# mindspore-lab/mindaudio

Measured on AMD Instinct MI355X. Metric: utterances/s (16 kHz×10 s) fbanks+Conformer fwd, 1/2/4/8 MI355X, higher is better.
Workload: dtype bf16; 1 GPU; features.fbank (n_fft=512 hop=160 n_mels=80, batch-global top_db) on 64 x (10 s @16 kHz) synthetic waves per GPU -> Conformer-small encoder forward (12 blocks, d=256, 4 heads, ff=2048, conv k=15, eval mode) on the (64, 1000, 80) features; random-init weights; global_batch=64, frames=1000

## Files before the change

mindaudio_amd/csrc/subsample_fused.hip:

```cpp
#include <hip/hip_runtime.h>
#include <stdint.h>
#include <stdlib.h>

#include <type_traits>
#include <utility>

#include "../../include/mindaudio_amd.h"

#include "launch.h"

namespace ma {

typedef __attribute__((ext_vector_type(8))) __bf16 sf_bf16x8;
typedef __attribute__((ext_vector_type(4))) float sf_f32x4;
typedef __attribute__((ext_vector_type(2))) __bf16 sf_bf16x2;
typedef __attribute__((ext_vector_type(2))) float sf_f32x2;
typedef __attribute__((address_space(3))) void sf_lds_void_t;

template <int... Is, class F>
__device__ __forceinline__ void sf_static_for_impl(std::integer_sequence<int, Is...>, F&& f) {
  (f(std::integral_constant<int, Is>{}), ...);
}
template <int N, class F>
__device__ __forceinline__ void sf_static_for(F&& f) {
  sf_static_for_impl(std::make_integer_sequence<int, N>{}, f);
}

constexpr int kSfRows = 128, kSfC = 256, kSfThreads = 512;
constexpr int kSfIdim = 80, kSfF1 = 39, kSfF2 = 19;
constexpr int kSfNhoMax = 8;
constexpr int kSfH1Max = 2 * kSfNhoMax + 1;
constexpr int kSfInMax = 2 * kSfH1Max + 1;
constexpr int kSfPosMax = 672;
constexpr int kSfPitch = 80;
constexpr int kSfChunks = 8, kSfTaps = 9;
constexpr int kSfW2Bytes = kSfC * 9 * kSfC * 2;
constexpr int kSfOffX = 11264;
constexpr int kSfOffPatch = kSfOffX + kSfPosMax * 64;
constexpr int kSfPatchBytes = kSfPosMax * kSfPitch;
constexpr int kSfLds = kSfOffPatch + 2 * kSfPatchBytes;
constexpr int kSfOutPitch = 144;
static_assert(kSfInMax * kSfIdim <= 6 * kSfThreads && kSfPosMax <= 2 * kSfThreads && kSfLds <= 163840, "tile geometry");
static_assert(4 * kSfRows * kSfOutPitch <= kSfOffPatch + kSfPatchBytes, "epilogue staging must not reach patch buffer 1");

struct SubsampleFusedParams {
  const float* x;
  int64_t sb, st, sf;
  const float *mean, *istd;
  const char* packed;
  const float* b1;
  const float* b2;
  uint16_t* out;
  int32_t Ho, tiles_per_utt;
};

__device__ __forceinline__ uint32_t sf_pack_bf16(float lo, float hi) {
  const sf_bf16x2 r = __builtin_convertvector((sf_f32x2){lo, hi}, sf_bf16x2);
  return *reinterpret_cast<const uint32_t*>(&r);
}
__device__ __forceinline__ float sf_head(float x) { return __uint_as_float(sf_pack_bf16(x, 0.0f) << 16); }

template <bool IS_W>
__device__ __forceinline__ void sf_split_row(const float (&v)[9], uint32_t (&d)[16]) {
  float h[9], l[9];
#pragma unroll
  for (int t = 0; t < 9; ++t) {
    h[t] = sf_head(v[t]);
    l[t] = v[t] - h[t];
  }
  float k[32];
#pragma unroll
  for (int t = 0; t < 9; ++t) {
    k[t] = h[t];
    k[9 + t] = IS_W ? l[t] : h[t];
    k[18 + t] = IS_W ? h[t] : l[t];
  }
#pragma unroll
  for (int t = 27; t < 32; ++t) k[t] = 0.0f;
#pragma unroll
  for (int j = 0; j < 16; ++j) d[j] = sf_pack_bf16(k[2 * j], k[2 * j + 1]);
}

__global__ void subsample_fused_pack_kernel(const uint16_t* __restrict__ w2, const float* __restrict__ w1, uint4* __restrict__ out) {
  const int idx = blockIdx.x * blockDim.x + threadIdx.x;
  constexpr int kN2 = 4 * kSfChunks * kSfTaps * 4 * 64;
  if (idx < kN2) {
    const int lane = idx & 63, jt = (idx >> 6) & 3, ft = (idx >> 8) % (kSfChunks * kSfTaps), wv = (idx >> 8) / (kSfChunks * kSfTaps);
    const int cc = ft / kSfTaps, tap = ft - cc * kSfTaps;
    const int n = 64 * wv + 16 * jt + (lane & 15);
    out[idx] = *reinterpret_cast<const uint4*>(w2 + (int64_t)n * (9 * kSfC) + tap * kSfC + 32 * cc + 8 * (lane >> 4));
  } else if (idx < kN2 + 16 * 64) {
    const int j = idx - kN2, lane = j & 63, item = j >> 6;
    const int ch = 16 * item + (lane & 15), g = lane >> 4;
    float v[9];
#pragma unroll
    for (int t = 0; t < 9; ++t) v[t] = w1[ch * 9 + t];
    uint32_t d[16];
    sf_split_row<true>(v, d);
    out[idx] = g == 0 ? make_uint4(d[0], d[1], d[2], d[3]) : g == 1 ? make_uint4(d[4], d[5], d[6], d[7])
             : g == 2 ? make_uint4(d[8], d[9], d[10], d[11]) : make_uint4(d[12], d[13], d[14], d[15]);
  }
}

#ifndef SF_PRIO_C
#define SF_PRIO_C 1
#endif
#ifndef SF_PRIO_P
#define SF_PRIO_P 0
#endif
#ifdef MA_SF_PROF
__device__ unsigned long long g_sf_prof[2 * 3 * 32];
#define SF_STAMP(k) do { asm volatile("s_waitcnt lgkmcnt(0)" ::: "memory"); sf_ts[(k)] = __builtin_amdgcn_s_memtime(); asm volatile("s_waitcnt lgkmcnt(0)" ::: "memory"); } while (0)
#define SF_FLUSH(role)                                                                                        \
  do {                                                                                                        \
    const int slot_ = blockIdx.x == 0 ? 0 : blockIdx.x == 1200 ? 1 : blockIdx.x == 2300 ? 2 : -1;             \
    if (slot_ >= 0 && lane == 0)                                                                              \
      for (int k_ = 0; k_ < 32; ++k_) g_sf_prof[((role) * 3 + slot_) * 32 + k_] = sf_ts[k_];                  \
  } while (0)
#else
#define SF_STAMP(k) do { } while (0)
#define SF_FLUSH(role) do { } while (0)
#endif

__global__ __launch_bounds__(kSfThreads, 2) void subsample_fused_kernel(const SubsampleFusedParams p) {
  extern __shared__ __attribute__((aligned(16))) char smem[];
#ifdef MA_SF_PROF
  unsigned long long sf_ts[32] = {};
#endif
  SF_STAMP(0);
  const int tid = threadIdx.x, lane = tid & 63;
  const int wave = __builtin_amdgcn_readfirstlane(tid >> 6);
  const int b = blockIdx.x / p.tiles_per_utt, ti = blockIdx.x - b * p.tiles_per_utt;
  const int npos = p.Ho * kSfF2;
  const int p0 = ti * kSfRows;
  const int np = min(kSfRows, npos - p0);
  const int ho0 = p0 / kSfF2;
  const int nho = (p0 + np - 1) / kSfF2 - ho0 + 1;
  const int nh1 = 2 * nho + 1, nin = 2 * nh1 + 1;
  const int npatch = nh1 * kSfF1;
  float* rows = reinterpret_cast<float*>(smem);
  char* xim = smem + kSfOffX;
  char* patch = smem + kSfOffPatch;

  {
    const float* xb = p.x + (int64_t)b * p.sb + (int64_t)(4 * ho0) * p.st;
    const bool tfast = p.st <= p.sf;
    const int n = nin * kSfIdim;
    float v[6], mu[6], is[6];
    int dst[6];
#pragma unroll
    for (int j = 0; j < 6; ++j) {
      const int i = min(tid + kSfThreads * j, n - 1);
      const int r = tfast ? i % nin : i / kSfIdim, f = tfast ? i / nin : i % kSfIdim;
      dst[j] = r * kSfIdim + f;
      v[j] = xb[r * p.st + f * p.sf];
      mu[j] = p.mean ? p.mean[f] : 0.0f;
      is[j] = p.mean ? p.istd[f] : 1.0f;
    }
#pragma unroll
    for (int j = 0; j < 6; ++j)
      if (tid + kSfThreads * j < n) rows[dst[j]] = p.mean ? (v[j] - mu[j]) * is[j] : v[j];
  }
  __syncthreads();
  SF_STAMP(1);
#pragma unroll
  for (int j = 0; j < 2; ++j) {
    const int pos = tid + kSfThreads * j;
    if (pos < kSfPosMax) {
      uint32_t d[16];
      if (pos < npatch) {
        const int h = pos / kSfF1, w = pos - h * kSfF1;
        const float* in = rows + (2 * h) * kSfIdim + 2 * w;
        float v[9];
#pragma unroll
        for (int kh = 0; kh < 3; ++kh)
#pragma unroll
          for (int kw = 0; kw < 3; ++kw) v[kh * 3 + kw] = in[kh * kSfIdim + kw];
        sf_split_row<false>(v, d);
      } else {
#pragma unroll
        for (int q = 0; q < 16; ++q) d[q] = 0u;
      }
      uint4* xo = reinterpret_cast<uint4*>(xim + pos * 64);
      xo[0] = make_uint4(d[0], d[1], d[2], d[3]);
      xo[1] = make_uint4(d[4], d[5], d[6], d[7]);
      xo[2] = make_uint4(d[8], d[9], d[10], d[11]);
      xo[3] = make_uint4(d[12], d[13], d[14], d[15]);
    }
  }
  __syncthreads();
  SF_STAMP(2);

  const int ci = lane & 15, gi = lane >> 4;
  auto build_patch = [&](int cc, int pw, int nprod) __attribute__((always_inline)) {
    const uint4* w1f = reinterpret_cast<const uint4*>(p.packed + kSfW2Bytes) + (2 * cc) * 64 + lane;
    const uint4 wa = w1f[0], wb = w1f[64];
    const sf_bf16x8 a0 = *reinterpret_cast<const sf_bf16x8*>(&wa), a1 = *reinterpret_cast<const sf_bf16x8*>(&wb);
    const float4 ba = *reinterpret_cast<const float4*>(p.b1 + 32 * cc + 4 * gi);
    const float4 bb = *reinterpret_cast<const float4*>(p.b1 + 32 * cc + 16 + 4 * gi);
    const sf_f32x4 c0 = {ba.x, ba.y, ba.z, ba.w}, c1 = {bb.x, bb.y, bb.z, bb.w};
    const char* xsrc = xim + ci * 64 + gi * 16;
    char* dst = patch + (cc & 1) * kSfPatchBytes + ci * kSfPitch + gi * 8;
    const int ntile = (npatch + 15) >> 4;
    for (int pt = pw; pt < ntile; pt += nprod) {
      const uint4 xr = *reinterpret_cast<const uint4*>(xsrc + pt * (16 * 64));
      const sf_bf16x8 xf = *reinterpret_cast<const sf_bf16x8*>(&xr);
      const sf_f32x4 d0 = __builtin_amdgcn_mfma_f32_16x16x32_bf16(a0, xf, c0, 0, 0, 0);
      const sf_f32x4 d1 = __builtin_amdgcn_mfma_f32_16x16x32_bf16(a1, xf, c1, 0, 0, 0);
      char* o = dst + pt * (16 * kSfPitch);
      *reinterpret_cast<uint2*>(o) = make_uint2(sf_pack_bf16(fmaxf(d0[0], 0.f), fmaxf(d0[1], 0.f)), sf_pack_bf16(fmaxf(d0[2], 0.f), fmaxf(d0[3], 0.f)));
      *reinterpret_cast<uint2*>(o + 32) = make_uint2(sf_pack_bf16(fmaxf(d1[0], 0.f), fmaxf(d1[1], 0.f)), sf_pack_bf16(fmaxf(d1[2], 0.f), fmaxf(d1[3], 0.f)));
    }
  };
  build_patch(0, wave, 8);
  SF_STAMP(3);

  if (wave >= 4) {
#if SF_PRIO_P
    __builtin_amdgcn_s_setprio(SF_PRIO_P);
#endif
#pragma unroll 1
    for (int k = 0; k + 1 < kSfChunks; ++k) {
      __syncthreads();
      SF_STAMP(4 + 2 * k);
      build_patch(k + 1, wave - 4, 4);
      SF_STAMP(5 + 2 * k);
    }
    __syncthreads();
    SF_STAMP(20);
    if (wave == 4) SF_FLUSH(1);
    return;
  }

#if SF_PRIO_C
  __builtin_amdgcn_s_setprio(SF_PRIO_C);
#endif
  const int c = lane & 15, g = lane >> 4;
  uint32_t a_addr[8];
#pragma unroll
  for (int s = 0; s < 8; ++s) {
    int m = 16 * s + c;
    if (m >= np) m = np - 1;
    const int pos = p0 + m, ho = pos / kSfF2, wo = pos - ho * kSfF2;
    a_addr[s] = (uint32_t)(uintptr_t)(sf_lds_void_t*)(patch + ((2 * (ho - ho0)) * kSfF1 + 2 * wo) * kSfPitch + g * 16);
  }
  const uint32_t voff = lane * 16 + 2048;
  const char* wbase = p.packed + (int64_t)wave * (kSfChunks * kSfTaps) * 4096;
#define SF_LOAD(dst, ft, jt)                                                                                          \
  do {                                                                                                                \
    const char* cb_ = wbase + (int64_t)((ft) < kSfChunks * kSfTaps ? (ft) : kSfChunks * kSfTaps - 1) * 4096;          \
    asm volatile("global_load_dwordx4 %0, %1, %2 offset:%3" : "=v"(dst) : "v"(voff), "s"(cb_), "n"(((jt) - 2) * 1024) \
                 : "memory");                                                                                         \
  } while (0)
  sf_bf16x8 ring[8];
  sf_f32x4 acc[4][8];
  sf_bf16x8 af[2][8];
#define SF_LDS(dst, s_, imm_) asm volatile("ds_read_b128 %0, %1 offset:%2" : "=v"(dst) : "v"(a_addr[s_]), "n"(imm_) : "memory")
#define SF_LDS8(buf_, imm_)                                                                                   \
  SF_LDS(af[buf_][0], 0, imm_); SF_LDS(af[buf_][1], 1, imm_); SF_LDS(af[buf_][2], 2, imm_); SF_LDS(af[buf_][3], 3, imm_); \
  SF_LDS(af[buf_][4], 4, imm_); SF_LDS(af[buf_][5], 5, imm_); SF_LDS(af[buf_][6], 6, imm_); SF_LDS(af[buf_][7], 7, imm_)
  auto tap_step = [&](auto tapc, auto parc, auto bufc, int ft) __attribute__((always_inline)) {
    constexpr int TAP = decltype(tapc)::value, PAR = decltype(parc)::value, BUF = decltype(bufc)::value;
    constexpr int IMM = BUF * kSfPatchBytes + ((TAP / 3) * kSfF1 + (TAP % 3)) * kSfPitch;
    constexpr int NTAP = TAP + 1;
    constexpr int IMM_N = BUF * kSfPatchBytes + ((NTAP / 3) * kSfF1 + (NTAP % 3)) * kSfPitch;
    if constexpr (TAP == 0) { SF_LDS8(PAR, IMM); }
    if constexpr (TAP < kSfTaps - 1) {
      SF_LDS8(PAR ^ 1, IMM_N);
      asm volatile("s_waitcnt lgkmcnt(8)"
                   : "+v"(af[PAR][0]), "+v"(af[PAR][1]), "+v"(af[PAR][2]), "+v"(af[PAR][3]), "+v"(af[PAR][4]), "+v"(af[PAR][5]),
                     "+v"(af[PAR][6]), "+v"(af[PAR][7])::"memory");
    } else {
      asm volatile("s_waitcnt lgkmcnt(0)"
                   : "+v"(af[PAR][0]), "+v"(af[PAR][1]), "+v"(af[PAR][2]), "+v"(af[PAR][3]), "+v"(af[PAR][4]), "+v"(af[PAR][5]),
                     "+v"(af[PAR][6]), "+v"(af[PAR][7])::"memory");
    }
    sf_static_for<4>([&](auto tc) __attribute__((always_inline)) {
      constexpr int jt = decltype(tc)::value;
      constexpr int q = PAR * 4 + jt;
      asm volatile("s_waitcnt vmcnt(7)" : "+v"(ring[q])::"memory");
      sf_static_for<8>([&](auto sc) __attribute__((always_inline)) {
        constexpr int s = decltype(sc)::value;
        acc[jt][s] = __builtin_amdgcn_mfma_f32_16x16x32_bf16(ring[q], af[PAR][s], acc[jt][s], 0, 0, 0);
      });
      __builtin_amdgcn_sched_barrier(0);
      SF_LOAD(ring[q], ft + 2, jt);
    });
  };
  auto chunk_mfma = [&](auto bufc, int cc) __attribute__((always_inline)) {
    constexpr int BUF = decltype(bufc)::value;
    sf_static_for<kSfTaps>([&](auto tapc) __attribute__((always_inline)) {
      constexpr int TAP = decltype(tapc)::value;
      tap_step(tapc, std::integral_constant<int, (BUF + TAP) & 1>{}, bufc, cc * kSfTaps + TAP);
    });
  };

#pragma unroll
  for (int jt = 0; jt < 4; ++jt)
#pragma unroll
    for (int s = 0; s < 8; ++s) acc[jt][s] = sf_f32x4{0.f, 0.f, 0.f, 0.f};
  SF_LOAD(ring[0], 0, 0); SF_LOAD(ring[1], 0, 1); SF_LOAD(ring[2], 0, 2); SF_LOAD(ring[3], 0, 3);
  SF_LOAD(ring[4], 1, 0); SF_LOAD(ring[5], 1, 1); SF_LOAD(ring[6], 1, 2); SF_LOAD(ring[7], 1, 3);
  asm volatile("s_waitcnt lgkmcnt(0)" ::: "memory");
  __builtin_amdgcn_s_barrier();
#ifdef MA_SF_PROF
#pragma unroll
#else
#pragma unroll 1
#endif
  for (int cc = 0; cc < kSfChunks; cc += 2) {
    SF_STAMP(4 + 2 * cc);
    chunk_mfma(std::integral_constant<int, 0>{}, cc);
    SF_STAMP(5 + 2 * cc);
    __builtin_amdgcn_s_barrier();
    SF_STAMP(6 + 2 * cc);
    chunk_mfma(std::integral_constant<int, 1>{}, cc + 1);
    SF_STAMP(7 + 2 * cc);
    if (cc + 2 < kSfChunks) __builtin_amdgcn_s_barrier();
  }
  asm volatile("s_waitcnt vmcnt(0)"
               : "+v"(ring[0]), "+v"(ring[1]), "+v"(ring[2]), "+v"(ring[3]), "+v"(ring[4]), "+v"(ring[5]), "+v"(ring[6]), "+v"(ring[7])
               :
               : "memory");
#undef SF_LOAD
#undef SF_LDS
#undef SF_LDS8
  SF_STAMP(20);

  char* strip = smem + wave * (kSfRows * kSfOutPitch);
  float4 bv[4];
#pragma unroll
  for (int jt = 0; jt < 4; ++jt) bv[jt] = *reinterpret_cast<const float4*>(p.b2 + 64 * wave + 16 * jt + 4 * g);
#pragma unroll
  for (int s = 0; s < 8; ++s) {
    char* srow = strip + (16 * s + c) * kSfOutPitch + 8 * g;
#pragma unroll
    for (int jt = 0; jt < 4; ++jt) {
      const float v0 = fmaxf(acc[jt][s][0] + bv[jt].x, 0.f), v1 = fmaxf(acc[jt][s][1] + bv[jt].y, 0.f);
      const float v2 = fmaxf(acc[jt][s][2] + bv[jt].z, 0.f), v3 = fmaxf(acc[jt][s][3] + bv[jt].w, 0.f);
      *reinterpret_cast<uint2*>(srow + 32 * jt) = make_uint2(sf_pack_bf16(v0, v1), sf_pack_bf16(v2, v3));
    }
  }
  uint16_t* obase = p.out + ((int64_t)b * npos + p0) * kSfC + 64 * wave + 8 * (lane & 7);
#pragma unroll
  for (int it = 0; it < 16; ++it) {
    const int m = 8 * it + (lane >> 3);
    const uint4 v = *reinterpret_cast<const uint4*>(strip + m * kSfOutPitch + 16 * (lane & 7));
    if (m < np) *reinterpret_cast<uint4*>(obase + (int64_t)m * kSfC) = v;
  }
  SF_STAMP(21);
  if (wave == 0) SF_FLUSH(0);
}

#ifdef MA_SF_PROF
extern "C" int ma_debug_sf_prof(unsigned long long* host192) {
  return hipMemcpyFromSymbol(host192, HIP_SYMBOL(g_sf_prof), sizeof(unsigned long long) * 192) == hipSuccess ? 0 : -1;
}
#endif

MA_LDS_ATTR(subsample_fused_kernel, kSfLds);

}

using namespace ma;

extern "C" int64_t ma_subsample_fused_packed_bytes(int64_t idim, int64_t C) {
  if (idim != kSfIdim || C != kSfC) return MA_ERR_UNSUPPORTED;
  return (int64_t)kSfW2Bytes + 16 * 1024;
}

extern "C" int ma_subsample_fused_pack_bf16(const float* W1, const void* W2, int64_t idim, int64_t C, void* packed, ma_stream_t stream) {
  if (!W1 || !W2 || !packed) return MA_ERR_INVALID_ARG;
  if (ma_subsample_fused_packed_bytes(idim, C) < 0) return MA_ERR_UNSUPPORTED;
  if ((reinterpret_cast<uintptr_t>(W2) | reinterpret_cast<uintptr_t>(packed)) & 15) return MA_ERR_INVALID_ARG;
  const int total = 4 * kSfChunks * kSfTaps * 4 * 64 + 16 * 64;
  MA_LAUNCH(subsample_fused_pack_kernel, dim3((total + 255) / 256), dim3(256), 0, (hipStream_t)stream,
            reinterpret_cast<const uint16_t*>(W2), W1, reinterpret_cast<uint4*>(packed));
  return MA_OK;
}

extern "C" int ma_subsample_fused_bf16(const float* x, int64_t stride_b, int64_t stride_t, int64_t stride_f, int64_t batch, int64_t T,
                                       int32_t idim, const float* cmvn_mean, const float* cmvn_istd, const void* packed, const float* b1,
                                       const float* b2, int64_t C, void* out, ma_stream_t stream) {
  if (!x || !packed || !b1 || !b2 || !out || batch < 1 || T < 7) return MA_ERR_INVALID_ARG;
  if ((cmvn_mean == nullptr) != (cmvn_istd == nullptr)) return MA_ERR_INVALID_ARG;
  if (ma_subsample_fused_packed_bytes(idim, C) < 0) return MA_ERR_UNSUPPORTED;
  if ((reinterpret_cast<uintptr_t>(packed) | reinterpret_cast<uintptr_t>(out) | reinterpret_cast<uintptr_t>(b2) |
       reinterpret_cast<uintptr_t>(b1)) & 15)
    return MA_ERR_INVALID_ARG;
  const int64_t T1 = (T - 3) / 2 + 1, Ho = (T1 - 3) / 2 + 1;
  const int64_t tiles = (Ho * kSfF2 + kSfRows - 1) / kSfRows;
  if (batch * tiles > 0x7fffffff || Ho > (1 << 24)) return MA_ERR_UNSUPPORTED;
  SubsampleFusedParams p;
  p.x = x;
  p.sb = stride_b;
  p.st = stride_t;
  p.sf = stride_f;
  p.mean = cmvn_mean;
  p.istd = cmvn_istd;
  p.packed = reinterpret_cast<const char*>(packed);
  p.b1 = b1;
  p.b2 = b2;
  p.out = reinterpret_cast<uint16_t*>(out);
  p.Ho = (int32_t)Ho;
  p.tiles_per_utt = (int32_t)tiles;
  MA_LAUNCH(subsample_fused_kernel, dim3((unsigned)(batch * tiles)), dim3(kSfThreads), kSfLds, (hipStream_t)stream, p);
  return MA_OK;
}
```

Measured before the change: 33050 utterances/s.

## Make fused subsample conv a persistent kernel overlapping next-tile load with MFMA

Replaces the one-block-per-tile subsample conv kernel with a persistent kernel launched at most once per CU. Each block walks a contiguous range of 16-row granules, so tile sizes are balanced across blocks. The producer waves load and normalise the next tile's input rows while still building patches for the current tile, and the consumer waves keep their weight ring loads flowing across tiles. The second conv's bias is staged in LDS and the epilogue is written in two halves. This aims to cut launch tail imbalance and the per-tile prologue stalls, at the cost of more register pressure and more complex synchronisation. The old tile kernel stays available behind an environment variable.

```diff
diff --git a/mindaudio_amd/csrc/subsample_fused.hip b/mindaudio_amd/csrc/subsample_fused.hip
--- a/mindaudio_amd/csrc/subsample_fused.hip
+++ b/mindaudio_amd/csrc/subsample_fused.hip
@@ -52,6 +52,8 @@
   const float* b2;
   uint16_t* out;
   int32_t Ho, tiles_per_utt;
+  int32_t gran_per_utt;
+  int64_t gran_total;
 };
 
 __device__ __forceinline__ uint32_t sf_pack_bf16(float lo, float hi) {
@@ -79,6 +81,99 @@
   for (int t = 27; t < 32; ++t) k[t] = 0.0f;
 #pragma unroll
   for (int j = 0; j < 16; ++j) d[j] = sf_pack_bf16(k[2 * j], k[2 * j + 1]);
+}
+
+struct SfGeom {
+  int ho0, nin, npatch;
+};
+__device__ __forceinline__ SfGeom sf_geom(int p0, int np) {
+  const int ho0 = p0 / kSfF2;
+  const int nho = (p0 + np - 1) / kSfF2 - ho0 + 1;
+  const int nh1 = 2 * nho + 1;
+  return {ho0, 2 * nh1 + 1, nh1 * kSfF1};
+}
+
+template <int J>
+struct SfRowsRegs {
+  float v[J], mu[J], is[J];
+  int dst[J];
+};
+template <int NT, int J>
+__device__ __forceinline__ void sf_rows_load(const SubsampleFusedParams& p, int b, const SfGeom& q, int t, SfRowsRegs<J>& r) {
+  static_assert(kSfInMax * kSfIdim <= NT * J, "rows staging");
+  const float* xb = p.x + (int64_t)b * p.sb + (int64_t)(4 * q.ho0) * p.st;
+  const bool tfast = p.st <= p.sf;
+  const int n = q.nin * kSfIdim;
+#pragma unroll
+  for (int j = 0; j < J; ++j) {
+    const int i = min(t + NT * j, n - 1);
+    const int rr = tfast ? i % q.nin : i / kSfIdim, f = tfast ? i / q.nin : i % kSfIdim;
+    r.dst[j] = rr * kSfIdim + f;
+    r.v[j] = xb[rr * p.st + f * p.sf];
+    r.mu[j] = p.mean ? p.mean[f] : 0.0f;
+    r.is[j] = p.mean ? p.istd[f] : 1.0f;
+  }
+}
+template <int NT, int J>
+__device__ __forceinline__ void sf_rows_store(const SubsampleFusedParams& p, const SfGeom& q, int t, const SfRowsRegs<J>& r, float* rows) {
+  const int n = q.nin * kSfIdim;
+#pragma unroll
+  for (int j = 0; j < J; ++j)
+    if (t + NT * j < n) rows[r.dst[j]] = p.mean ? (r.v[j] - r.mu[j]) * r.is[j] : r.v[j];
+}
+
+__device__ __forceinline__ void sf_build_x(const float* rows, char* xim, int pos, int npatch) {
+  uint32_t d[16];
+  if (pos < npatch) {
+    const int h = pos / kSfF1, w = pos - h * kSfF1;
+    const float* in = rows + (2 * h) * kSfIdim + 2 * w;
+    float v[9];
+#pragma unroll
+    for (int kh = 0; kh < 3; ++kh)
+#pragma unroll
+      for (int kw = 0; kw < 3; ++kw) v[kh * 3 + kw] = in[kh * kSfIdim + kw];
+    sf_split_row<false>(v, d);
+  } else {
+#pragma unroll
+    for (int q = 0; q < 16; ++q) d[q] = 0u;
+  }
+  uint4* xo = reinterpret_cast<uint4*>(xim + pos * 64);
+  xo[0] = make_uint4(d[0], d[1], d[2], d[3]);
+  xo[1] = make_uint4(d[4], d[5], d[6], d[7]);
+  xo[2] = make_uint4(d[8], d[9], d[10], d[11]);
+  xo[3] = make_uint4(d[12], d[13], d[14], d[15]);
+}
+
+struct SfW1 {
+  sf_bf16x8 a0, a1;
+  sf_f32x4 c0, c1;
+};
+__device__ __forceinline__ SfW1 sf_patch_w1(const SubsampleFusedParams& p, int cc, int lane) {
+  const int gi = lane >> 4;
+  const uint4* w1f = reinterpret_cast<const uint4*>(p.packed + kSfW2Bytes) + (2 * cc) * 64 + lane;
+  const uint4 wa = w1f[0], wb = w1f[64];
+  const float4 ba = *reinterpret_cast<const float4*>(p.b1 + 32 * cc + 4 * gi);
+  const float4 bb = *reinterpret_cast<const float4*>(p.b1 + 32 * cc + 16 + 4 * gi);
+  return {*reinterpret_cast<const sf_bf16x8*>(&wa), *reinterpret_cast<const sf_bf16x8*>(&wb), sf_f32x4{ba.x, ba.y, ba.z, ba.w},
+          sf_f32x4{bb.x, bb.y, bb.z, bb.w}};
+}
+__device__ __forceinline__ void sf_build_patch(const SfW1& w, const char* xim, char* patch, int npatch, int cc, int pw, int nprod,
+                                               int lane) {
+  const int ci = lane & 15, gi = lane >> 4;
+  const sf_bf16x8 a0 = w.a0, a1 = w.a1;
+  const sf_f32x4 c0 = w.c0, c1 = w.c1;
+  const char* xsrc = xim + ci * 64 + gi * 16;
+  char* dst = patch + (cc & 1) * kSfPatchBytes + ci * kSfPitch + gi * 8;
+  const int ntile = (npatch + 15) >> 4;
+  for (int pt = pw; pt < ntile; pt += nprod) {
+    const uint4 xr = *reinterpret_cast<const uint4*>(xsrc + pt * (16 * 64));
+    const sf_bf16x8 xf = *reinterpret_cast<const sf_bf16x8*>(&xr);
+    const sf_f32x4 d0 = __builtin_amdgcn_mfma_f32_16x16x32_bf16(a0, xf, c0, 0, 0, 0);
+    const sf_f32x4 d1 = __builtin_amdgcn_mfma_f32_16x16x32_bf16(a1, xf, c1, 0, 0, 0);
+    char* o = dst + pt * (16 * kSfPitch);
+    *reinterpret_cast<uint2*>(o) = make_uint2(sf_pack_bf16(fmaxf(d0[0], 0.f), fmaxf(d0[1], 0.f)), sf_pack_bf16(fmaxf(d0[2], 0.f), fmaxf(d0[3], 0.f)));
+    *reinterpret_cast<uint2*>(o + 32) = make_uint2(sf_pack_bf16(fmaxf(d1[0], 0.f), fmaxf(d1[1], 0.f)), sf_pack_bf16(fmaxf(d1[2], 0.f), fmaxf(d1[3], 0.f)));
+  }
 }
 
 __global__ void subsample_fused_pack_kernel(const uint16_t* __restrict__ w2, const float* __restrict__ w1, uint4* __restrict__ out) {
@@ -122,7 +217,7 @@
 #define SF_FLUSH(role) do { } while (0)
 #endif
 
-__global__ __launch_bounds__(kSfThreads, 2) void subsample_fused_kernel(const SubsampleFusedParams p) {
+__global__ __launch_bounds__(kSfThreads, 2) void subsample_fused_tile_kernel(const SubsampleFusedParams p) {
   extern __shared__ __attribute__((aligned(16))) char smem[];
 #ifdef MA_SF_PROF
   unsigned long long sf_ts[32] = {};
@@ -134,85 +229,26 @@
   const int npos = p.Ho * kSfF2;
   const int p0 = ti * kSfRows;
   const int np = min(kSfRows, npos - p0);
-  const int ho0 = p0 / kSfF2;
-  const int nho = (p0 + np - 1) / kSfF2 - ho0 + 1;
-  const int nh1 = 2 * nho + 1, nin = 2 * nh1 + 1;
-  const int npatch = nh1 * kSfF1;
+  const SfGeom q = sf_geom(p0, np);
+  const int npatch = q.npatch;
   float* rows = reinterpret_cast<float*>(smem);
   char* xim = smem + kSfOffX;
   char* patch = smem + kSfOffPatch;
 
   {
-    const float* xb = p.x + (int64_t)b * p.sb + (int64_t)(4 * ho0) * p.st;
-    const bool tfast = p.st <= p.sf;
-    const int n = nin * kSfIdim;
-    float v[6], mu[6], is[6];
-    int dst[6];
-#pragma unroll
-    for (int j = 0; j < 6; ++j) {
-      const int i = min(tid + kSfThreads * j, n - 1);
-      const int r = tfast ? i % nin : i / kSfIdim, f = tfast ? i / nin : i % kSfIdim;
-      dst[j] = r * kSfIdim + f;
-      v[j] = xb[r * p.st + f * p.sf];
-      mu[j] = p.mean ? p.mean[f] : 0.0f;
-      is[j] = p.mean ? p.istd[f] : 1.0f;
-    }
-#pragma unroll
-    for (int j = 0; j < 6; ++j)
-      if (tid + kSfThreads * j < n) rows[dst[j]] = p.mean ? (v[j] - mu[j]) * is[j] : v[j];
+    SfRowsRegs<6> r;
+    sf_rows_load<kSfThreads, 6>(p, b, q, tid, r);
+    sf_rows_store<kSfThreads, 6>(p, q, tid, r, rows);
   }
   __syncthreads();
   SF_STAMP(1);
 #pragma unroll
-  for (int j = 0; j < 2; ++j) {
-    const int pos = tid + kSfThreads * j;
-    if (pos < kSfPosMax) {
-      uint32_t d[16];
-      if (pos < npatch) {
-        const int h = pos / kSfF1, w = pos - h * kSfF1;
-        const float* in = rows + (2 * h) * kSfIdim + 2 * w;
-        float v[9];
-#pragma unroll
-        for (int kh = 0; kh < 3; ++kh)
-#pragma unroll
-          for (int kw = 0; kw < 3; ++kw) v[kh * 3 + kw] = in[kh * kSfIdim + kw];
-        sf_split_row<false>(v, d);
-      } else {
-#pragma unroll
-        for (int q = 0; q < 16; ++q) d[q] = 0u;
-      }
-      uint4* xo = reinterpret_cast<uint4*>(xim + pos * 64);
-      xo[0] = make_uint4(d[0], d[1], d[2], d[3]);
-      xo[1] = make_uint4(d[4], d[5], d[6], d[7]);
-      xo[2] = make_uint4(d[8], d[9], d[10], d[11]);
-      xo[3] = make_uint4(d[12], d[13], d[14], d[15]);
-    }
-  }
+  for (int j = 0; j < 2; ++j)
+    if (tid + kSfThreads * j < kSfPosMax) sf_build_x(rows, xim, tid + kSfThreads * j, npatch);
   __syncthreads();
   SF_STAMP(2);
 
-  const int ci = lane & 15, gi = lane >> 4;
-  auto build_patch = [&](int cc, int pw, int nprod) __attribute__((always_inline)) {
-    const uint4* w1f = reinterpret_cast<const uint4*>(p.packed + kSfW2Bytes) + (2 * cc) * 64 + lane;
-    const uint4 wa = w1f[0], wb = w1f[64];
-    const sf_bf16x8 a0 = *reinterpret_cast<const sf_bf16x8*>(&wa), a1 = *reinterpret_cast<const sf_bf16x8*>(&wb);
-    const float4 ba = *reinterpret_cast<const float4*>(p.b1 + 32 * cc + 4 * gi);
-    const float4 bb = *reinterpret_cast<const float4*>(p.b1 + 32 * cc + 16 + 4 * gi);
-    const sf_f32x4 c0 = {ba.x, ba.y, ba.z, ba.w}, c1 = {bb.x, bb.y, bb.z, bb.w};
-    const char* xsrc = xim + ci * 64 + gi * 16;
-    char* dst = patch + (cc & 1) * kSfPatchBytes + ci * kSfPitch + gi * 8;
-    const int ntile = (npatch + 15) >> 4;
-    for (int pt = pw; pt < ntile; pt += nprod) {
-      const uint4 xr = *reinterpret_cast<const uint4*>(xsrc + pt * (16 * 64));
-      const sf_bf16x8 xf = *reinterpret_cast<const sf_bf16x8*>(&xr);
-      const sf_f32x4 d0 = __builtin_amdgcn_mfma_f32_16x16x32_bf16(a0, xf, c0, 0, 0, 0);
-      const sf_f32x4 d1 = __builtin_amdgcn_mfma_f32_16x16x32_bf16(a1, xf, c1, 0, 0, 0);
-      char* o = dst + pt * (16 * kSfPitch);
-      *reinterpret_cast<uint2*>(o) = make_uint2(sf_pack_bf16(fmaxf(d0[0], 0.f), fmaxf(d0[1], 0.f)), sf_pack_bf16(fmaxf(d0[2], 0.f), fmaxf(d0[3], 0.f)));
-      *reinterpret_cast<uint2*>(o + 32) = make_uint2(sf_pack_bf16(fmaxf(d1[0], 0.f), fmaxf(d1[1], 0.f)), sf_pack_bf16(fmaxf(d1[2], 0.f), fmaxf(d1[3], 0.f)));
-    }
-  };
-  build_patch(0, wave, 8);
+  sf_build_patch(sf_patch_w1(p, 0, lane), xim, patch, npatch, 0, wave, 8, lane);
   SF_STAMP(3);
 
   if (wave >= 4) {
@@ -223,7 +259,7 @@
     for (int k = 0; k + 1 < kSfChunks; ++k) {
       __syncthreads();
       SF_STAMP(4 + 2 * k);
-      build_patch(k + 1, wave - 4, 4);
+      sf_build_patch(sf_patch_w1(p, k + 1, lane), xim, patch, npatch, k + 1, wave - 4, 4, lane);
       SF_STAMP(5 + 2 * k);
     }
     __syncthreads();
@@ -242,7 +278,7 @@
     int m = 16 * s + c;
     if (m >= np) m = np - 1;
     const int pos = p0 + m, ho = pos / kSfF2, wo = pos - ho * kSfF2;
-    a_addr[s] = (uint32_t)(uintptr_t)(sf_lds_void_t*)(patch + ((2 * (ho - ho0)) * kSfF1 + 2 * wo) * kSfPitch + g * 16);
+    a_addr[s] = (uint32_t)(uintptr_t)(sf_lds_void_t*)(patch + ((2 * (ho - q.ho0)) * kSfF1 + 2 * wo) * kSfPitch + g * 16);
   }
   const uint32_t voff = lane * 16 + 2048;
   const char* wbase = p.packed + (int64_t)wave * (kSfChunks * kSfTaps) * 4096;
@@ -352,17 +388,242 @@
   if (wave == 0) SF_FLUSH(0);
 }
 
+constexpr int kSfOffBias = kSfLds;
+constexpr int kSfLdsP = kSfOffBias + kSfC * 4;
+static_assert(kSfLdsP <= 163840 && 4 * 64 * kSfOutPitch <= kSfPatchBytes, "persistent LDS layout");
+
+struct SfTile {
+  int b, p0, np;
+};
+__device__ __forceinline__ SfTile sf_tile_at(const SubsampleFusedParams& p, int npos, int64_t& g, int64_t gend) {
+  const int b = (int)(g / p.gran_per_utt);
+  const int lg = (int)(g - (int64_t)b * p.gran_per_utt);
+  const int ng = (int)min((int64_t)(kSfRows / 16), min(gend - g, (int64_t)(p.gran_per_utt - lg)));
+  g += ng;
+  return {b, 16 * lg, min(16 * ng, npos - 16 * lg)};
+}
+
+__global__ __launch_bounds__(kSfThreads, 2) void subsample_fused_kernel(const SubsampleFusedParams p) {
+  extern __shared__ __attribute__((aligned(16))) char smem[];
+  const int tid = threadIdx.x, lane = tid & 63;
+  const int wave = __builtin_amdgcn_readfirstlane(tid >> 6);
+  const int npos = p.Ho * kSfF2;
+  int64_t g = (int64_t)blockIdx.x * p.gran_total / gridDim.x;
+  const int64_t gend = (int64_t)(blockIdx.x + 1) * p.gran_total / gridDim.x;
+  float* rows = reinterpret_cast<float*>(smem);
+  char* xim = smem + kSfOffX;
+  char* patch = smem + kSfOffPatch;
+  float* bias2 = reinterpret_cast<float*>(smem + kSfOffBias);
+
+  SfTile t = sf_tile_at(p, npos, g, gend);
+  SfGeom q = sf_geom(t.p0, t.np);
+  {
+    SfRowsRegs<6> r;
+    sf_rows_load<kSfThreads, 6>(p, t.b, q, tid, r);
+    if (tid < kSfC) bias2[tid] = p.b2[tid];
+    sf_rows_store<kSfThreads, 6>(p, q, tid, r, rows);
+  }
+  __syncthreads();
+#pragma unroll
+  for (int j = 0; j < 2; ++j)
+    if (tid + kSfThreads * j < kSfPosMax) sf_build_x(rows, xim, tid + kSfThreads * j, q.npatch);
+  __syncthreads();
+  sf_build_patch(sf_patch_w1(p, 0, lane), xim, patch, q.npatch, 0, wave, 8, lane);
+
+  if (wave >= 4) {
+#if SF_PRIO_P
+    __builtin_amdgcn_s_setprio(SF_PRIO_P);
+#endif
+    const int pw = wave - 4, ptid = tid - 4 * 64;
+    for (;;) {
+      const bool more = g < gend;
+      const SfTile tn = more ? sf_tile_at(p, npos, g, gend) : t;
+      const SfGeom qn = sf_geom(tn.p0, tn.np);
+      __syncthreads();
+      const SfW1 w1 = sf_patch_w1(p, 1, lane);
+      SfRowsRegs<11> r;
+      if (more) sf_rows_load<4 * 64, 11>(p, tn.b, qn, ptid, r);
+      sf_build_patch(w1, xim, patch, q.npatch, 1, pw, 4, lane);
+      if (more) sf_rows_store<4 * 64, 11>(p, qn, ptid, r, rows);
+#pragma unroll 1
+      for (int k = 1; k + 1 < kSfChunks; ++k) {
+        __syncthreads();
+        sf_build_patch(sf_patch_w1(p, k + 1, lane), xim, patch, q.npatch, k + 1, pw, 4, lane);
+      }
+      __syncthreads();
+      if (more) {
+#pragma unroll
+        for (int j = 0; j < 3; ++j) {
+          const int pos = 16 * (pw + 4 * ((lane >> 4) + 4 * j)) + (lane & 15);
+          if (pos < kSfPosMax) sf_build_x(rows, xim, pos, qn.npatch);
+        }
+      }
+      __syncthreads();
+      if (!more) return;
+      sf_build_patch(sf_patch_w1(p, 0, lane), xim, patch, qn.npatch, 0, pw, 4, lane);
+      t = tn;
+      q = qn;
+    }
+  }
+
+#if SF_PRIO_C
+  __builtin_amdgcn_s_setprio(SF_PRIO_C);
+#endif
+  const uint32_t voff = lane * 16 + 2048;
+  const char* wbase = p.packed + (int64_t)wave * (kSfChunks * kSfTaps) * 4096;
+#define SF_LOAD(dst, ft, jt)                                                                                          \
+  do {                                                                                                                \
+    const char* cb_ = wbase + (int64_t)((ft) < kSfChunks * kSfTaps ? (ft) : (ft) - kSfChunks * kSfTaps) * 4096;       \
+    asm volatile("global_load_dwordx4 %0, %1, %2 offset:%3" : "=v"(dst) : "v"(voff), "s"(cb_), "n"(((jt) - 2) * 1024) \
+                 : "memory");                                                                                         \
+  } while (0)
+  sf_bf16x8 ring[8];
+  sf_f32x4 acc[4][8];
+  sf_bf16x8 af[2][8];
+  uint32_t a_addr[8];
+#define SF_LDS(dst, s_, imm_) asm volatile("ds_read_b128 %0, %1 offset:%2" : "=v"(dst) : "v"(a_addr[s_]), "n"(imm_) : "memory")
+#define SF_LDS8(buf_, imm_)                                                                                   \
+  SF_LDS(af[buf_][0], 0, imm_); SF_LDS(af[buf_][1], 1, imm_); SF_LDS(af[buf_][2], 2, imm_); SF_LDS(af[buf_][3], 3, imm_); \
+  SF_LDS(af[buf_][4], 4, imm_); SF_LDS(af[buf_][5], 5, imm_); SF_LDS(af[buf_][6], 6, imm_); SF_LDS(af[buf_][7], 7, imm_)
+  auto tap_step = [&](auto tapc, auto parc, auto bufc, int ft) __attribute__((always_inline)) {
+    constexpr int TAP = decltype(tapc)::value, PAR = decltype(parc)::value, BUF = decltype(bufc)::value;
+    constexpr int IMM = BUF * kSfPatchBytes + ((TAP / 3) * kSfF1 + (TAP % 3)) * kSfPitch;
+    constexpr int NTAP = TAP + 1;
+    constexpr int IMM_N = BUF * kSfPatchBytes + ((NTAP / 3) * kSfF1 + (NTAP % 3)) * kSfPitch;
+    if constexpr (TAP == 0) { SF_LDS8(PAR, IMM); }
+    if constexpr (TAP < kSfTaps - 1) {
+      SF_LDS8(PAR ^ 1, IMM_N);
+      asm volatile("s_waitcnt lgkmcnt(8)"
+                   : "+v"(af[PAR][0]), "+v"(af[PAR][1]), "+v"(af[PAR][2]), "+v"(af[PAR][3]), "+v"(af[PAR][4]), "+v"(af[PAR][5]),
+                     "+v"(af[PAR][6]), "+v"(af[PAR][7])::"memory");
+    } else {
+      asm volatile("s_waitcnt lgkmcnt(0)"
+                   : "+v"(af[PAR][0]), "+v"(af[PAR][1]), "+v"(af[PAR][2]), "+v"(af[PAR][3]), "+v"(af[PAR][4]), "+v"(af[PAR][5]),
+                     "+v"(af[PAR][6]), "+v"(af[PAR][7])::"memory");
+    }
+    sf_static_for<4>([&](auto tc) __attribute__((always_inline)) {
+      constexpr int jt = decltype(tc)::value;
+      constexpr int qr = PAR * 4 + jt;
+      asm volatile("s_waitcnt vmcnt(7)" : "+v"(ring[qr])::"memory");
+      sf_static_for<8>([&](auto sc) __attribute__((always_inline)) {
+        constexpr int s = decltype(sc)::value;
+        acc[jt][s] = __builtin_amdgcn_mfma_f32_16x16x32_bf16(ring[qr], af[PAR][s], acc[jt][s], 0, 0, 0);
+      });
+      __builtin_amdgcn_sched_barrier(0);
+      SF_LOAD(ring[qr], ft + 2, jt);
+    });
+  };
+  auto chunk_mfma = [&](auto bufc, int cc) __attribute__((always_inline)) {
+    constexpr int BUF = decltype(bufc)::value;
+    sf_static_for<kSfTaps>([&](auto tapc) __attribute__((always_inline)) {
+      constexpr int TAP = decltype(tapc)::value;
+      tap_step(tapc, std::integral_constant<int, (BUF + TAP) & 1>{}, bufc, cc * kSfTaps + TAP);
+    });
+  };
+  SF_LOAD(ring[0], 0, 0); SF_LOAD(ring[1], 0, 1); SF_LOAD(ring[2], 0, 2); SF_LOAD(ring[3], 0, 3);
+  SF_LOAD(ring[4], 1, 0); SF_LOAD(ring[5], 1, 1); SF_LOAD(ring[6], 1, 2); SF_LOAD(ring[7], 1, 3);
+  char* strip = patch + kSfPatchBytes + wave * (64 * kSfOutPitch);
+  for (;;) {
+    const bool more = g < gend;
+    const SfTile tn = more ? sf_tile_at(p, npos, g, gend) : t;
+    int ln = lane;
+    asm volatile("" : "+v"(ln));
+    const int c = ln & 15, gq = ln >> 4;
+#pragma unroll
+    for (int s = 0; s < 8; ++s) {
+      int m = 16 * s + c;
+      if (m >= t.np) m = t.np - 1;
+      const int pos = t.p0 + m, ho = pos / kSfF2, wo = pos - ho * kSfF2;
+      a_addr[s] = (uint32_t)(uintptr_t)(sf_lds_void_t*)(patch + ((2 * (ho - q.ho0)) * kSfF1 + 2 * wo) * kSfPitch + gq * 16);
+    }
+#pragma unroll
+    for (int jt = 0; jt < 4; ++jt)
+#pragma unroll
+      for (int s = 0; s < 8; ++s) acc[jt][s] = sf_f32x4{0.f, 0.f, 0.f, 0.f};
+    asm volatile("s_waitcnt lgkmcnt(0)" ::: "memory");
+    __builtin_amdgcn_s_barrier();
+#pragma unroll 1
+    for (int cc = 0; cc < kSfChunks; cc += 2) {
+      chunk_mfma(std::integral_constant<int, 0>{}, cc);
+      __builtin_amdgcn_s_barrier();
+      chunk_mfma(std::integral_constant<int, 1>{}, cc + 1);
+      if (cc + 2 < kSfChunks) __builtin_amdgcn_s_barrier();
+    }
+    __builtin_amdgcn_s_barrier();
+
+    int le = lane;
+    asm volatile("" : "+v"(le));
+    const int ce = le & 15, ge = le >> 4;
+    float4 bv[4];
+#pragma unroll
+    for (int jt = 0; jt < 4; ++jt) bv[jt] = *reinterpret_cast<const float4*>(bias2 + 64 * wave + 16 * jt + 4 * ge);
+    uint16_t* obase = p.out + ((int64_t)t.b * npos + t.p0) * kSfC + 64 * wave + 8 * (le & 7);
+#pragma unroll
+    for (int hh = 0; hh < 2; ++hh) {
+      if (hh == 1 && t.np <= 64) break;
+#pragma unroll
+      for (int s = 4 * hh; s < 4 * hh + 4; ++s) {
+        char* srow = strip + (16 * (s - 4 * hh) + ce) * kSfOutPitch + 8 * ge;
+#pragma unroll
+        for (int jt = 0; jt < 4; ++jt) {
+          const float v0 = fmaxf(acc[jt][s][0] + bv[jt].x, 0.f), v1 = fmaxf(acc[jt][s][1] + bv[jt].y, 0.f);
+          const float v2 = fmaxf(acc[jt][s][2] + bv[jt].z, 0.f), v3 = fmaxf(acc[jt][s][3] + bv[jt].w, 0.f);
+          *reinterpret_cast<uint2*>(srow + 32 * jt) = make_uint2(sf_pack_bf16(v0, v1), sf_pack_bf16(v2, v3));
+        }
+      }
+#pragma unroll
+      for (int it = 0; it < 8; ++it) {
+        const int m = 8 * it + (le >> 3);
+        const uint4 v = *reinterpret_cast<const uint4*>(strip + m * kSfOutPitch + 16 * (le & 7));
+        if (64 * hh + m < t.np) *reinterpret_cast<uint4*>(obase + (int64_t)(64 * hh + m) * kSfC) = v;
+      }
+    }
+    if (!more) break;
+    t = tn;
+    q = sf_geom(t.p0, t.np);
+  }
+  asm volatile("s_waitcnt vmcnt(0)"
+               : "+v"(ring[0]), "+v"(ring[1]), "+v"(ring[2]), "+v"(ring[3]), "+v"(ring[4]), "+v"(ring[5]), "+v"(ring[6]), "+v"(ring[7])
+               :
+               : "memory");
+#undef SF_LOAD
+#undef SF_LDS
+#undef SF_LDS8
+}
+
+
 #ifdef MA_SF_PROF
 extern "C" int ma_debug_sf_prof(unsigned long long* host192) {
   return hipMemcpyFromSymbol(host192, HIP_SYMBOL(g_sf_prof), sizeof(unsigned long long) * 192) == hipSuccess ? 0 : -1;
 }
 #endif
 
-MA_LDS_ATTR(subsample_fused_kernel, kSfLds);
+MA_LDS_ATTR(subsample_fused_tile_kernel, kSfLds);
+MA_LDS_ATTR(subsample_fused_kernel, kSfLdsP);
 
 }
 
 using namespace ma;
+
+static bool subsample_use_tile() {
+  static const bool use = [] {
+    const char* e = getenv("MINDAUDIO_AMD_SUBSAMPLE");
+    return e && e[0] == 't' && e[1] == 'i' && e[2] == 'l' && e[3] == 'e' && e[4] == 0;
+  }();
+  return use;
+}
+
+static int subsample_cu_count() {
+  constexpr int kMaxDev = 64;
+  static int cached[kMaxDev] = {};
+  int dev = 0;
+  if (hipGetDevice(&dev) != hipSuccess) return -1;
+  if (dev >= 0 && dev < kMaxDev && cached[dev] > 0) return cached[dev];
+  int n = 0;
+  if (hipDeviceGetAttribute(&n, hipDeviceAttributeMultiprocessorCount, dev) != hipSuccess || n < 1) return -1;
+  if (dev >= 0 && dev < kMaxDev) cached[dev] = n;
+  return n;
+}
 
 extern "C" int64_t ma_subsample_fused_packed_bytes(int64_t idim, int64_t C) {
   if (idim != kSfIdim || C != kSfC) return MA_ERR_UNSUPPORTED;
@@ -404,6 +665,14 @@
   p.out = reinterpret_cast<uint16_t*>(out);
   p.Ho = (int32_t)Ho;
   p.tiles_per_utt = (int32_t)tiles;
-  MA_LAUNCH(subsample_fused_kernel, dim3((unsigned)(batch * tiles)), dim3(kSfThreads), kSfLds, (hipStream_t)stream, p);
+  p.gran_per_utt = (int32_t)((Ho * kSfF2 + 15) / 16);
+  p.gran_total = batch * p.gran_per_utt;
+  if (subsample_use_tile()) {
+    MA_LAUNCH(subsample_fused_tile_kernel, dim3((unsigned)(batch * tiles)), dim3(kSfThreads), kSfLds, (hipStream_t)stream, p);
+    return MA_OK;
+  }
+  const int cus = subsample_cu_count();
+  if (cus < 1) return MA_ERR_LAUNCH;
+  MA_LAUNCH(subsample_fused_kernel, dim3((unsigned)min(batch * tiles, (int64_t)cus)), dim3(kSfThreads), kSfLdsP, (hipStream_t)stream, p);
   return MA_OK;
 }
```

Result: no change. 33230 utterances/s, median of 6 (+0.6%).
